# jmscraig/deequ

Measured on AMD Instinct MI355X. Metric: rows/sec + achieved HBM GB/s, fused 10-analyzer suite on 1B rows, 1/2/4/8 GPUs, higher is better.
Workload: dtype int64; 1 GPU; S10 fused suite (Size, Completeness(id), Completeness(name), Compliance(numViews >= 0), Compliance(priority IS NULL OR priority IN ('high','low')), Sum/Mean/StandardDeviation/Minimum/Maximum(numViews)) over a synthetic Item table: int64 id/numViews, string name/priority, 5% nulls (BASELINE.json configs[1]); rows_per_gpu=1000000000, batch_rows=67108864, parallelism=dp1

## Files before the change

### deequ_amd/csrc/api.cpp

```cpp
#include <hip/hip_runtime.h>

#include <algorithm>
#include <cmath>
#include <cstdarg>
#include <cstdio>
#include <cstdlib>
#include <cstring>
#include <map>
#include <mutex>
#include <memory>
#include <string>
#include <tuple>
#include <vector>

#include "decimal.h"
#include "engine.h"
#include "kernels.h"
#include "jfmt.h"

using namespace dq;

#include <atomic>
static std::atomic<long long> g_host_waits{0};
static hipError_t host_wait(hipStream_t st) {
// ... 391 lines not shown
  int op = n.op;
  auto is_lit = [](const Node* x) { return x->op == DQ_X_I64 || x->op == DQ_X_F64; };
  auto colref = [&](const Node* x) -> int {
    if (x->op == DQ_X_COL && is_numeric(types[x->col])) return x->col;
    return -1;
  };
  if (colref(b) >= 0 && is_lit(a)) {
    std::swap(a, b);
    op = flip_cmp(op);
  }
  int c = colref(a);
  if (c < 0 || !is_lit(b)) return false;
  out.col = c;
  out.op = op;
  out.lit_f64 = b->op == DQ_X_F64;
  out.li = b->i;
  out.ld = b->op == DQ_X_F64 ? b->d : (double)b->i;
  return true;
}

static bool fuse_numeric(const Node& n, const std::vector<int32_t>& types, int& col, NumPred& p) {
  p = NumPred{};
  if (interpreter_only(n)) return false;
  const Node* body = &n;
  int null_col = -1;
  if (n.op == DQ_X_OR && n.kids[0]->op == DQ_X_IS_NULL && n.kids[0]->kids[0]->op == DQ_X_COL) {
    null_col = n.kids[0]->kids[0]->col;
    body = n.kids[1].get();
  }
  CmpLeaf a, b;
  bool two = false;
  if (body->op == DQ_X_AND) {
    if (!leaf_cmp(*body->kids[0], types, a) || !leaf_cmp(*body->kids[1], types, b)) return false;
    if (a.col != b.col) return false;
    two = true;
  } else if (!leaf_cmp(*body, types, a)) {
    return false;
  }
  if (null_col >= 0 && null_col != a.col) return false;
  const bool fcol = is_floating(types[a.col]);
  const bool as_double = fcol || a.lit_f64 || (two && b.lit_f64);
  if (two && !fcol && (a.lit_f64 != b.lit_f64)) return false;
  if (as_double && !fcol && types[a.col] == DQ_INT64) {
  }
  col = a.col;
  p.op1 = a.op;
  p.op2 = two ? b.op : 0;
  p.as_double = as_double ? 1 : 0;
  p.null_is_true = null_col >= 0 ? 1 : 0;
  p.lo_i = a.li;
  p.lo_d = a.ld;
  p.hi_i = two ? b.li : 0;
  p.hi_d = two ? b.ld : 0.0;
  return true;
}

struct StrIn {
  int col = -1;
  bool negate = false;
  bool null_is_true = false;
  std::vector<std::string> list;
};

static bool fuse_str_in_body(const Node& n, const std::vector<int32_t>& types, StrIn& s) {
  if (n.op == DQ_X_NOT) {
    if (!fuse_str_in_body(*n.kids[0], types, s)) return false;
    s.negate = !s.negate;
    return true;
  }
  if (n.op == DQ_X_IN) {
    const Node& x = *n.kids[0];
    if (x.op != DQ_X_COL || types[x.col] != DQ_UTF8) return false;
    for (size_t k = 1; k < n.kids.size(); ++k) {
      if (n.kids[k]->op != DQ_X_STR) return false;
      s.list.push_back(n.kids[k]->s);
    }
    s.col = x.col;
    return true;
  }
  if (n.op == DQ_X_EQ || n.op == DQ_X_NE) {
    const Node* a = n.kids[0].get();
    const Node* b = n.kids[1].get();
    if (a->op == DQ_X_STR) std::swap(a, b);
    if (a->op != DQ_X_COL || types[a->col] != DQ_UTF8 || b->op != DQ_X_STR) return false;
    s.col = a->col;
    s.list.push_back(b->s);
    s.negate = n.op == DQ_X_NE;
    return true;
  }
  return false;
}

static bool fuse_str_in(const Node& n, const std::vector<int32_t>& types, StrIn& s) {
  s = StrIn{};
  if (interpreter_only(n)) return false;
  if (n.op == DQ_X_OR && n.kids[0]->op == DQ_X_IS_NULL && n.kids[0]->kids[0]->op == DQ_X_COL) {
    int nc = n.kids[0]->kids[0]->col;
    if (!fuse_str_in_body(*n.kids[1], types, s)) return false;
    if (s.col != nc) return false;
    s.null_is_true = true;
    return true;
  }
  return fuse_str_in_body(n, types, s);
}

enum SlotSrc { SRC_ROWS = 1, SRC_TASK = 2 };
// ... 338 lines not shown
  s += line;
  size_t n = std::min(buf_len - 1, s.size());
  memcpy(buf, s.data(), n);
  buf[n] = '\0';
  return DQ_OK;
}

extern "C" int dq_plan_launches_per_batch(const dq_plan* plan) {
  if (!plan) return 0;
  int classes = 0, hll = 0;
  for (int c = 0; c < kBodyClasses; ++c) {
    bool used = false;
    for (const TaskPlan& t : plan->tasks) used = used || (body_class(plan, t) == c && !t.carried);
    if (c == BC_HLL || c == BC_CORR_HLL || c == BC_DECIMAL) hll += used ? 1 : 0;
    else classes += used ? 1 : 0;
  }
  bool hll_alone = false;
  for (const TaskPlan& t : plan->tasks) hll_alone = hll_alone || (t.kind == TK_HLL && !t.carried);
  if (hll_alone && plan->n_hll <= kMixedHllMax && classes >= 1) {
    classes += 1;
    hll -= 1;
  }
  if (classes >= 2 && !getenv("DQ_NO_MIXED")) classes = 1;
  return (int)plan->mat.size() + classes + hll + (plan->tasks.empty() ? 0 : 1);
}

struct dq_state {
  const dq_plan* plan = nullptr;
  int device = 0;
  int grid[kQueues] = {};
  int mix_hll = 0;
  hipStream_t stream = nullptr;
  bool stream_set = false;
  std::vector<Acc> acc;
  std::vector<uint8_t> hll;
  int64_t rows = 0;
  bool host_dirty = false;
  bool reset_pending = false;
  bool synced = true;
  void* h_pin = nullptr;
  size_t h_pin_cap = 0;
  bool pin_pending = false;
  DevBuf<Acc> d_acc, d_partial, d_partial2;
  DevBuf<uint8_t> d_hll;
  DevBuf<uint32_t> d_hll_stage;
  DevBuf<uint32_t> d_fin_arrivals;
  DevBuf<int64_t> d_rows;
  DevBuf<int32_t> d_kinds;
  std::vector<int32_t> h_kinds;
  bool kinds_ready = false;
  hipEvent_t ev_xchg = nullptr;
  bool rows_on_device = false;
  DevBuf<uint32_t> d_queue;
  DevBuf<uint32_t> d_order[2];
  std::vector<uint32_t> order_sig[2];
  std::vector<size_t> order_off[2], order_len[2];
  uint32_t* h_order[2] = {nullptr, nullptr};
  size_t h_order_cap[2] = {0, 0};
  DevBuf<TaskDesc> d_tasks[2];
  TaskDesc* h_tasks[2] = {nullptr, nullptr};
  size_t h_tasks_cap[2] = {0, 0};
  hipEvent_t ev[2] = {nullptr, nullptr};
  bool ev_used[2] = {false, false};
  int flip = 0;
  DevBuf<uint64_t> d_bitmaps;
  size_t bitmap_words = 0;
  DevBuf<XInstr> d_prog;
  std::vector<int> prog_off;
  DevBuf<uint8_t> d_pool;
  std::vector<int64_t> pool_off;
  struct RegexRun {
    int col = -1, null_mode = 0, ns = 0, start = 0;
    int64_t table_off = 0;
  };
  std::vector<RegexRun> rx;
  DevBuf<DevCol> d_cols[2];
  DevCol* h_cols[2] = {nullptr, nullptr};
  size_t h_cols_cap[2] = {0, 0};
  DevBuf<int32_t> d_list_i32;
  DevBuf<uint64_t> d_list_pre;
  DevBuf<uint8_t> d_list_bytes;
  std::vector<int64_t> list_i32_base, list_pre_base, list_byte_base;
  ~dq_state() {
    for (int k = 0; k < 2; ++k) {
      if (h_tasks[k]) (void)hipHostFree(h_tasks[k]);
      if (h_cols[k]) (void)hipHostFree(h_cols[k]);
      if (h_order[k]) (void)hipHostFree(h_order[k]);
      if (ev[k]) (void)hipEventDestroy(ev[k]);
    }
    if (ev_xchg) (void)hipEventDestroy(ev_xchg);
  }
};

static void host_reset(dq_state* s) {
  const dq_plan* p = s->plan;
  s->acc.assign(p->tasks.size(), Acc{});
  for (size_t k = 0; k < p->tasks.size(); ++k) acc_init(p->tasks[k].kind, s->acc[k]);
  s->hll.assign((size_t)p->n_hll * kHllM, 0);
  s->rows = 0;
  s->host_dirty = true;
  s->synced = true;
}

static dq_status pin_ensure(dq_state* s, size_t bytes) {
  if (s->h_pin_cap >= bytes) return DQ_OK;
  if (s->pin_pending) {
    HIP_TRY(host_wait(s->stream));
    s->pin_pending = false;
  }
  if (s->h_pin) (void)hipHostFree(s->h_pin);
// ... 243 lines not shown
    }
    if (!ref[c]) continue;
    if (cols[c].length < 0) {
      st = fail(DQ_ERR_INVALID_ARGUMENT, "negative column length");
      return -1;
    }
    if (rows < 0) rows = cols[c].length;
    else if (rows != cols[c].length) {
      st = fail(DQ_ERR_INVALID_ARGUMENT, "columns of one batch differ in length");
      return -1;
    }
    if (cols[c].length > 0 && !cols[c].values) {
      st = fail(DQ_ERR_INVALID_ARGUMENT, "column %zu has no values buffer", c);
      return -1;
    }
    if (cols[c].type == DQ_UTF8 && cols[c].length > 0 && !cols[c].data) {
      st = fail(DQ_ERR_INVALID_ARGUMENT, "utf8 column %zu has no data buffer", c);
      return -1;
    }
  }
  if (rows < 0) rows = plan->types.empty() ? 0 : cols[0].length;
  if (rows > ((int64_t)1 << 40)) {
    st = fail(DQ_ERR_UNSUPPORTED, "batch too large");
    return -1;
  }
  return rows;
}

extern "C" dq_status dq_scan_device(const dq_plan* plan, const dq_column* cols, int n_cols,
                                    dq_state* s, void* hip_stream) {
  return dq_scan_device_batches(plan, cols, n_cols, 1, s, hip_stream);
}

constexpr int64_t kTailDiv = 32;
constexpr int64_t kTailCut = 8;
constexpr int64_t kTailMinItems = 16;
static bool tail_split() {
  static const bool on = [] {
    const char* e = getenv("DQ_TAIL_SPLIT");
    return !e || atoi(e) != 0;
  }();
  return on;
}

static bool scan_has_tail(const TaskDesc* td, size_t n_desc, const ScanLaunch& L) {
  for (size_t q = 0; q < n_desc; ++q)
    if (td[q].n_items > td[q].n_big && (uint32_t)td[q].item_begin >= L.item_lo &&
        (uint32_t)td[q].item_begin < L.item_hi)
      return true;
  return false;
}

static void scan_order(const TaskDesc* td, size_t n_desc, const std::vector<ScanLaunch>& G,
                       std::vector<uint32_t>& out) {
  std::vector<std::vector<uint32_t>> big(G.size()), small(G.size());
  for (size_t c = 0; c < G.size(); ++c)
    for (size_t q = 0; q < n_desc; ++q) {
      const TaskDesc& t = td[q];
      if (t.n_items == 0 || (uint32_t)t.item_begin < G[c].item_lo || (uint32_t)t.item_begin >= G[c].item_hi)
        continue;
      for (int64_t i = 0; i < t.n_items; ++i)
        (i < t.n_big ? big[c] : small[c]).push_back((uint32_t)(t.item_begin + i));
    }
  auto interleave = [](std::vector<std::vector<uint32_t>>& lists) {
    std::vector<uint32_t> r;
    std::vector<size_t> next(lists.size(), 0);
    size_t total = 0;
    for (auto& l : lists) total += l.size();
    r.reserve(total);
    for (size_t k = 0; k < total; ++k) {
      int best = -1;
      double best_key = 0.0;
      for (size_t c = 0; c < lists.size(); ++c) {
        if (next[c] >= lists[c].size()) continue;
        const double key = (next[c] + 0.5) / (double)lists[c].size();
        if (best < 0 || key < best_key) {
          best = (int)c;
          best_key = key;
        }
      }
      r.push_back(lists[best][next[best]++]);
    }
    return r;
  };
  const std::vector<uint32_t> B = interleave(big), S = interleave(small);
  const uint64_t n = B.size() + S.size();
  size_t bi = 0, si = 0;
  for (int x = 0; x < kQueueHeads; ++x) {
    const uint64_t len = n * (x + 1) / kQueueHeads - n * x / kQueueHeads;
    const uint64_t want_s = (uint64_t)S.size() * (x + 1) / kQueueHeads - (uint64_t)si;
    uint64_t ns = std::min<uint64_t>(want_s, len), nb = len - ns;
    if (nb > B.size() - bi) {
      nb = B.size() - bi;
      ns = len - nb;
    }
    for (uint64_t k = 0; k < nb; ++k) out.push_back(B[bi++]);
    for (uint64_t k = 0; k < ns; ++k) out.push_back(S[si++]);
  }
}

extern "C" dq_status dq_scan_device_batches(const dq_plan* plan, const dq_column* cols, int n_cols,
                                            int n_batches, dq_state* s, void* hip_stream) {
  if (!plan || !s || (n_cols > 0 && n_batches > 0 && !cols))
    return fail(DQ_ERR_INVALID_ARGUMENT, "null argument");
  if (n_batches < 0) return fail(DQ_ERR_INVALID_ARGUMENT, "negative batch count");
  if (s->plan != plan) return fail(DQ_ERR_STATE, "state was created for another plan");
  if (n_cols < (int)plan->types.size())
    return fail(DQ_ERR_NO_SUCH_COLUMN, "plan needs %zu columns, got %d", plan->types.size(), n_cols);
  if (n_batches == 0) return DQ_OK;
  if (s->device < 0) return fail(DQ_ERR_STATE, "host-only state (device -1) cannot scan");
  hipStream_t stream = reinterpret_cast<hipStream_t>(hip_stream);
  HIP_TRY(hipSetDevice(s->device));
  if (s->rows_on_device) {
    const dq_status rs = dq_state_sync(s);
    if (rs != DQ_OK) return rs;
  }
  if (s->stream_set && s->stream != stream) HIP_TRY(host_wait(s->stream));
  s->stream = stream;
  s->stream_set = true;
  dq_status st = upload_host(s);
  if (st != DQ_OK) return st;

  std::vector<int> ref(plan->types.size(), 0);
  for (const TaskPlan& t : plan->tasks) {
    if (t.col >= 0) ref[t.col] = 1;
    if (t.col2 >= 0) ref[t.col2] = 1;
  }
  for (const MatExpr& m : plan->mat)
    for (const XInstr& ins : m.prog)
      if (ins.op == XI_COL) ref[ins.a] = 1;
  std::vector<int64_t> rows(n_batches);
  int64_t total_rows = 0;
  for (int b = 0; b < n_batches; ++b) {
    rows[b] = batch_rows(plan, cols + (size_t)b * n_cols, ref, st);
    if (rows[b] < 0) return st;
    total_rows += rows[b];
  }

// ... 157 lines not shown
      item_rows = std::max<int64_t>(kItemAlign, std::min<int64_t>(item_rows, (int64_t)1 << 22));
      t.item_rows = item_rows;
      t.n_items = rows[b] > 0 && !tp.carried ? (rows[b] + item_rows - 1) / item_rows : 0;
      t.n_big = t.n_items;
      t.small_rows = item_rows;
      if (tail_split() && t.n_items >= kTailMinItems && item_rows >= kTailCut * kItemAlign) {
        const int64_t k = (t.n_items + kTailDiv - 1) / kTailDiv;
        t.n_big = t.n_items - k;
        t.small_rows = item_rows / kTailCut;
        t.n_items = t.n_big + (rows[b] - t.n_big * item_rows + t.small_rows - 1) / t.small_rows;
      }
      t.item_begin = total_items;
      total_items += t.n_items;
      td[d] = t;
    }
    const int c = body_class(plan, tp);
    if (launches.empty() || launches.back().body != c)
      launches.push_back(ScanLaunch{c, s->grid[c], (uint32_t)td[d - n_batches].item_begin, 0, nullptr});
    launches.back().item_hi = (uint32_t)total_items;
  }
  if (total_items >= ((int64_t)1 << 31))
    return fail(DQ_ERR_UNSUPPORTED, "scan of %lld work items exceeds one launch",
                (long long)total_items);
  {
    std::vector<ScanLaunch> plain, hll;
    for (const ScanLaunch& L : launches)
      ((L.body == BC_HLL && !s->mix_hll) || L.body == BC_CORR_HLL || L.body == BC_DECIMAL ? hll : plain)
          .push_back(L);
    const bool mixed = plain.size() >= 2 && !getenv("DQ_NO_MIXED");
    if (mixed && plain.front().item_lo != 0) return fail(DQ_ERR_STATE, "unexpected item layout");
    std::vector<std::vector<ScanLaunch>> groups;
    if (mixed) groups.push_back(plain);
    else
      for (const ScanLaunch& L : plain) groups.push_back({L});
    for (const ScanLaunch& L : hll) groups.push_back({L});
    std::vector<uint32_t> sig;
    for (size_t q = 0; q < n_desc; ++q) {
      sig.push_back((uint32_t)td[q].item_begin);
      sig.push_back((uint32_t)td[q].n_big);
      sig.push_back((uint32_t)td[q].n_items);
    }
    for (const auto& G : groups) {
      sig.push_back(0xffffffffu);
      for (const ScanLaunch& L : G) {
        sig.push_back(L.item_lo);
        sig.push_back(L.item_hi);
      }
    }
    std::vector<size_t>& off = s->order_off[slot];
    std::vector<size_t>& len = s->order_len[slot];
    if (s->order_sig[slot] != sig) {
      off.assign(groups.size(), 0);
      len.assign(groups.size(), 0);
      std::vector<uint32_t> all;
      for (size_t g = 0; g < groups.size(); ++g) {
        off[g] = all.size();
        if (groups[g].size() >= 2 || scan_has_tail(td, n_desc, groups[g][0])) {
          scan_order(td, n_desc, groups[g], all);
          len[g] = all.size() - off[g];
        }
      }
      HIP_TRY(s->d_order[slot].ensure(std::max<size_t>(1, all.size())));
      if (!all.empty()) {
        if (s->h_order_cap[slot] < all.size()) {
          if (s->h_order[slot]) HIP_TRY(hipHostFree(s->h_order[slot]));
          s->h_order[slot] = nullptr;
          s->h_order_cap[slot] = 0;
          HIP_TRY(hipHostMalloc((void**)&s->h_order[slot], all.size() * sizeof(uint32_t),
                                hipHostMallocDefault));
          s->h_order_cap[slot] = all.size();
        }
        memcpy(s->h_order[slot], all.data(), all.size() * sizeof(uint32_t));
        HIP_TRY(hipMemcpyAsync(s->d_order[slot].p, s->h_order[slot], all.size() * sizeof(uint32_t),
                               hipMemcpyHostToDevice, stream));
      }
      s->order_sig[slot] = sig;
    }
    launches.clear();
    for (size_t g = 0; g < groups.size(); ++g) {
      const uint32_t* ord = len[g] ? s->d_order[slot].p + off[g] : nullptr;
      if (groups[g].size() >= 2) {
        bool has_hll = false;
        uint32_t classes = 0;
        for (const ScanLaunch& L : groups[g]) {
          has_hll = has_hll || L.body == BC_HLL;
          classes |= 1u << L.body;
        }
        launches.push_back(ScanLaunch{kBodyMixed, s->grid[kBodyMixed], 0, (uint32_t)len[g], ord,
                                      has_hll ? s->mix_hll : 0, classes});
      } else {
        ScanLaunch L = groups[g][0];
        if (ord) {
          L.item_lo = 0;
          L.item_hi = (uint32_t)len[g];
          L.order = ord;
        }
        launches.push_back(L);
      }
    }
  }
  if (getenv("DQ_DEBUG")) {
    for (const ScanLaunch& L : launches)
      fprintf(stderr, "[dq] launch body=%d grid=%d items=[%u,%u)\n", L.body, L.grid, L.item_lo,
              L.item_hi);
    for (size_t q = 0; q < n_desc; ++q)
      fprintf(stderr, "[dq] desc %zu kind=%d out=%d rows=%lld item_rows=%lld items=[%lld,+%lld) vec=%d\n",
              q, td[q].kind, td[q].out, (long long)td[q].rows, (long long)td[q].item_rows,
              (long long)td[q].item_begin, (long long)td[q].n_items, td[q].vec_ok);
  }
  if (n_desc > 0 && total_items > 0) {
    HIP_TRY(s->d_partial.ensure((size_t)total_items));
    HIP_TRY(hipMemcpyAsync(s->d_tasks[slot].p, td, n_desc * sizeof(TaskDesc), hipMemcpyHostToDevice,
                           stream));
    HIP_TRY(launch_scan(s->d_tasks[slot].p, (int)n_desc, (int)plan->tasks.size(), launches.data(),
                        (int)launches.size(), plan->n_hll, s->d_queue.p, s->d_partial.p,
                        s->d_partial2.p, s->d_hll_stage.p, s->d_acc.p, s->d_hll.p,
                        s->d_fin_arrivals.p, stream, s->reset_pending ? 1 : 0));
    s->reset_pending = false;
    s->synced = false;
  }
  HIP_TRY(hipEventRecord(s->ev[slot], stream));
  s->ev_used[slot] = true;
  s->rows += total_rows;
  return DQ_OK;
}

extern "C" dq_status dq_state_sync(dq_state* s) {
  if (!s) return fail(DQ_ERR_INVALID_ARGUMENT, "null state");
  if (s->synced || s->device < 0) return DQ_OK;
  HIP_TRY(hipSetDevice(s->device));
  const size_t ab = s->acc.size() * sizeof(Acc), hb = s->hll.size();
  const size_t rb = s->rows_on_device ? 8 : 0;
  {
// ... 817 lines not shown
```

### deequ_amd/csrc/engine.h

```cpp
#pragma once

#include <hip/hip_runtime.h>
#include <stdint.h>

#include "../../include/deequ_amd.h"

#define DQ_HD __host__ __device__ __forceinline__

namespace dq {

enum TaskKind : int32_t {
  TK_NUMERIC = 1,
  TK_VALIDITY = 2,
  TK_STR_IN = 3,
  TK_BOOLMAP = 4,
  TK_COMOMENTS = 5,
  TK_HLL = 6,
  TK_DTYPE = 7,
  TK_DECIMAL = 8
};

constexpr int kMaxPreds = 3;
constexpr int kHllP = 9;
constexpr int kHllM = 1 << kHllP;
constexpr int kHllWords = 52;
constexpr int kHllRegsPerWord = 10;
constexpr int kHllRegBits = 6;
constexpr int kBlock = 256;
constexpr int kWaveRows = 1024;
#ifndef DQ_ITEM_BYTES
#define DQ_ITEM_BYTES 262144
#endif
constexpr double kItemBytes = DQ_ITEM_BYTES;
constexpr int kItemAlign = 1024;
constexpr int kFinParts = 32;
constexpr int kListLenSlots = 65;

struct NumPred {
  int32_t op1, op2;
  int32_t as_double;
  int32_t null_is_true;
  int64_t lo_i, hi_i;
  double lo_d, hi_d;
};

struct TaskDesc {
  int32_t kind, type, type2, n_preds;
  int32_t out;
  int32_t hll_out;
  int32_t batch;
  int32_t negate;
  int32_t null_is_true;
  int32_t n_list;
  int32_t vec_ok;
  int32_t list_small;
  int32_t body;
  int32_t hll_side;
  uint64_t list_lenmask;
  uint64_t list_key[8];
  int64_t rows;
  int64_t item_rows;
  int64_t item_begin;
  int64_t n_items;
  int64_t n_big;
  int64_t small_rows;
  const uint8_t* valid;
  const void* values;
  const uint8_t* data;
  const uint8_t* valid2;
  const void* values2;
  const uint8_t* w_val;
  const uint8_t* w_vld;
  const uint8_t* b_val;
  const uint8_t* b_vld;
  const int32_t* list_start;
  const int32_t* list_len;
  const int32_t* list_boff;
  const uint64_t* list_pre;
  const uint8_t* list_bytes;
  NumPred preds[kMaxPreds];
};

struct alignas(16) Acc {
  int64_t i[10];
  double d[6];
};

DQ_HD void acc_init(int kind, Acc& a) {
  for (int k = 0; k < 10; ++k) a.i[k] = 0;
  for (int k = 0; k < 6; ++k) a.d[k] = 0.0;
  if (kind == TK_NUMERIC) {
    a.i[2] = INT64_MAX;
    a.i[3] = INT64_MIN;
  }
  if (kind == TK_DECIMAL) {
    a.i[4] = -1;
    a.i[5] = INT64_MAX;
// ... 288 lines not shown
```

### deequ_amd/csrc/kernels.h

```cpp
#pragma once

#include <hip/hip_runtime.h>
#include <stdint.h>

#include <string>
#include <utility>
#include <vector>

#include "engine.h"

namespace dq {

dq_status fail(dq_status code, const char* fmt, ...);

#define HIP_TRY(expr)                                                                        \
  do {                                                                                       \
    hipError_t _e = (expr);                                                                  \
    if (_e != hipSuccess) {                                                                  \
      return ::dq::fail(_e == hipErrorOutOfMemory ? DQ_ERR_OUT_OF_MEMORY : DQ_ERR_DEVICE,    \
                        "HIP error %s (%d) at %s:%d", hipGetErrorString(_e), (int)_e,        \
                        __FILE__, __LINE__);                                                 \
    }                                                                                        \
  } while (0)

// ... 86 lines not shown
  LK_ENDS,
  LK_ALL
};

struct XInstr {
  int32_t op;
  int32_t a;
  int64_t imm;
};

constexpr int kMaxStack = 16;

hipError_t launch_bitmap_rebase(const uint8_t* src, int64_t bit, int64_t rows, uint8_t* dst,
                                hipStream_t stream);
hipError_t launch_tile_scan(uint32_t* tiles, int64_t n, hipStream_t stream);
bool dict_index_type_ok(int index_type);
hipError_t launch_dict_count(const void* indices, int index_type, const uint8_t* valid, int64_t rows,
                             int64_t entries, unsigned long long* counts, unsigned long long* words,
                             hipStream_t stream);
hipError_t launch_expr(const XInstr* prog, int n_instr, const DevCol* cols, const uint8_t* pool,
                       int64_t rows, uint64_t* out_val, uint64_t* out_vld, hipStream_t stream);
constexpr int kRegexMaxStates = 255;
hipError_t launch_regex(const uint8_t* valid, const int32_t* offsets, const uint8_t* data,
                        int64_t rows, const uint8_t* table, int ns, int start, int null_mode,
                        uint64_t* out_val, uint64_t* out_vld, hipStream_t stream);
bool build_regex_table(const std::string& pool, int64_t at, std::vector<uint8_t>& tab, int* ns_out,
                       int* start_out);
enum BodyClass : int32_t {
  BC_NUM_I8 = 0,
  BC_NUM_I16,
  BC_NUM_I32,
  BC_NUM_I64,
  BC_NUM_F32,
  BC_NUM_F64,
  BC_BITS,
  BC_STR_IN,
  BC_DTYPE,
  BC_CORR,
  BC_HLL,
  BC_CORR_HLL,
  BC_DECIMAL,
  kBodyClasses
};
constexpr int kBodyMixed = kBodyClasses;
constexpr int kQueues = kBodyClasses + 1;
constexpr int kQueueHeads = 8;
constexpr int kQueueStride = 32;
constexpr int kQueueWords = kQueues * kQueueHeads * kQueueStride;

struct ScanLaunch {
  int32_t body;
  int32_t grid;
  uint32_t item_lo, item_hi;
  const uint32_t* order;
  int32_t lds_hll = 0;
  uint32_t classes = 0;
};
constexpr uint32_t kMixedAll = ((1u << kBodyClasses) - 1u) & ~(1u << BC_DECIMAL);
constexpr uint32_t kMixedS10 = (1u << BC_BITS) | (1u << BC_NUM_I64) | (1u << BC_STR_IN);

constexpr int kMixedHllMax = 0;

hipError_t launch_scan(const TaskDesc* tasks, int n_desc, int n_tasks, const ScanLaunch* launches,
                       int n_launches, int n_hll, uint32_t* queues, Acc* partial, Acc* partial2,
                       uint32_t* hll_stage, Acc* acc, uint8_t* hll_acc, uint32_t* arrivals,
                       hipStream_t stream, int reset = 0);
size_t scan_lds_bytes(int body, int n_hll);
int scan_max_blocks_per_cu(int body, int n_hll);
void plan_column_needs(const dq_plan* plan, std::vector<int>& need);

}
```

### deequ_amd/csrc/scan.hip

```cpp
#include <hip/hip_runtime.h>

#include <cstdlib>

#include "device_util.h"
#include "kernels.h"
#include "stream_load.h"

namespace dq {

DQ_DEV void wave_reduce(int kind, Acc& a) {
#pragma unroll
  for (int off = 32; off > 0; off >>= 1) {
    Acc o;
#pragma unroll
    for (int f = 0; f < 10; ++f) o.i[f] = __shfl_xor(a.i[f], off);
#pragma unroll
    for (int f = 0; f < 6; ++f) o.d[f] = __shfl_xor(a.d[f], off);
    acc_merge(kind, a, o);
  }
}

DQ_DEV uint32_t ld32_slow(const uint8_t* bm, int64_t word, int64_t rows) {
  if (!bm) return 0xffffffffu;
  uint32_t v = 0;
  for (int b = 0; b < 4; ++b) {
    int64_t byte = word * 4 + b;
    if (byte * 8 < rows) v |= (uint32_t)bm[byte] << (8 * b);
  }
  return v;
}

DQ_DEV bool near_constant(double m2b, int nb, double mb) {
  return m2b <= (double)nb * (mb * mb) * 0x1p-88;
}

template <int N, typename T>
DQ_DEV bool clamp_block_mean(const T* x, uint32_t sel, double& mb) {
  double lo = INFINITY, hi = -INFINITY;
#pragma unroll
  for (int i = 0; i < N; ++i) {
    const bool on = (sel >> i) & 1u;
    const double xd = (double)x[i];
    lo = (on && xd < lo) ? xd : lo;
    hi = (on && xd > hi) ? xd : hi;
  }
  const double c = mb < lo ? lo : (mb > hi ? hi : mb);
  const bool moved = c != mb;
  mb = c;
  return moved;
}

struct NumLane {
  int64_t n = 0, si = 0, kmin = INT64_MAX, kmax = INT64_MIN;
  double sd = 0.0, mean = 0.0, m2 = 0.0;
  uint32_t pt[kMaxPreds] = {0, 0, 0}, pn[kMaxPreds] = {0, 0, 0};
};

template <typename T>
DQ_DEV int64_t num_key(T v) {
  if constexpr (std::is_floating_point<T>::value) {
    return f64_key((double)v);
  } else {
    return (int64_t)v;
  }
}

template <typename T, int NV>
DQ_DEV uint32_t pred_bits(const NumPred& P, const T* x) {
  const uint32_t m1 = op_mask(P.op1), m2 = op_mask(P.op2);
  uint32_t r = 0;
  if (P.as_double) {
    const double lo = P.lo_d, hi = P.hi_d;
#pragma unroll
    for (int i = 0; i < NV; ++i) {
      const double xd = (double)x[i];
      uint32_t ok = (m1 >> (cmp3_f64(xd, lo) + 1)) & 1u;
      if (P.op2) ok &= (m2 >> (cmp3_f64(xd, hi) + 1)) & 1u;
      r |= ok << i;
    }
  } else {
    const int64_t lo = P.lo_i, hi = P.hi_i;
#pragma unroll
    for (int i = 0; i < NV; ++i) {
      const int64_t xi = (int64_t)x[i];
      uint32_t ok = (m1 >> (cmp3_i64(xi, lo) + 1)) & 1u;
      if (P.op2) ok &= (m2 >> (cmp3_i64(xi, hi) + 1)) & 1u;
      r |= ok << i;
    }
  }
  return r;
}

template <typename T, int NV>
DQ_DEV void num_vals(NumLane& L, const T* x, uint32_t vb, uint32_t wt, const TaskDesc& t) {
  const uint32_t sel = vb & wt;
  const int nb = __popc(sel);
  if (nb) {
    double s = 0.0;
#pragma unroll
    for (int i = 0; i < NV; ++i) {
      const bool on = (sel >> i) & 1u;
      if constexpr (!std::is_floating_point<T>::value) L.si = wrap_add(L.si, on ? (int64_t)x[i] : 0);
      s += on ? (double)x[i] : 0.0;
      const int64_t k = num_key(x[i]);
      L.kmin = (on && k < L.kmin) ? k : L.kmin;
      L.kmax = (on && k > L.kmax) ? k : L.kmax;
    }
    if constexpr (std::is_floating_point<T>::value) L.sd += s;
    double mb = s / (double)nb;
    double m2b = 0.0;
#pragma unroll
    for (int i = 0; i < NV; ++i) {
      const double d = (double)x[i] - mb;
      m2b += ((sel >> i) & 1u) ? d * d : 0.0;
    }
    if (near_constant(m2b, nb, mb) && clamp_block_mean<NV>(x, sel, mb)) {
      m2b = 0.0;
#pragma unroll
      for (int i = 0; i < NV; ++i) {
        const double d = (double)x[i] - mb;
        m2b += ((sel >> i) & 1u) ? d * d : 0.0;
      }
    }
    if (L.n == 0) {
      L.mean = mb;
      L.m2 = m2b;
    } else {
      moments_merge((double)L.n, L.mean, L.m2, (double)nb, mb, m2b);
    }
    L.n += nb;
  }
  if (t.n_preds == 0) return;
  const uint32_t nulls_all = wt & ~vb & ((1u << NV) - 1u);
#pragma unroll
  for (int p = 0; p < kMaxPreds; ++p) {
    if (p >= t.n_preds) break;
    const NumPred& P = t.preds[p];
    const uint32_t r = pred_bits<T, NV>(P, x);
    const uint32_t nulls = P.null_is_true ? nulls_all : 0u;
    L.pt[p] += __popc(r & sel) + __popc(nulls);
    L.pn[p] += __popc(sel) + __popc(nulls);
  }
}

template <typename T>
DQ_DEV void num_rows(NumLane& L, const T (&x)[16], uint32_t vb, uint32_t wt, const TaskDesc& t) {
  num_vals<T, 8>(L, x, vb & 0xffu, wt & 0xffu, t);
  num_vals<T, 8>(L, x + 8, vb >> 8, wt >> 8, t);
}

template <typename T>
DQ_DEV void num_chunk_fast(NumLane& L, const TaskDesc& t, int64_t r0) {
  constexpr int VPL = 16 / (int)sizeof(T);
  constexpr int U = 16 / VPL;
  const int l = lane_id();
  const T* v = reinterpret_cast<const T*>(t.values) + r0;
  uint4 raw[U];
#pragma unroll
  for (int k = 0; k < U; ++k) raw[k] = ld16(v + (k * 64 + l) * VPL);
  uint32_t vb = 0xffffu, wt = 0xffffu;
  if (t.valid) {
    ChunkBits c;
    c.load(t.valid, r0);
    vb = 0;
#pragma unroll
    for (int k = 0; k < U; ++k) vb |= c.get((k * 64 + l) * VPL, VPL) << (k * VPL);
  }
  if (t.w_val) {
    ChunkBits a, b;
    a.load(t.w_val, r0);
    b.load(t.w_vld, r0);
    wt = 0;
#pragma unroll
    for (int k = 0; k < U; ++k) {
      const int o = (k * 64 + l) * VPL;
      wt |= (a.get(o, VPL) & b.get(o, VPL)) << (k * VPL);
    }
  }
  T x[16];
  __builtin_memcpy(x, raw, sizeof(x));
  num_rows<T>(L, x, vb, wt, t);
}

template <typename T>
DQ_DEV void num_chunk_slow(NumLane& L, const TaskDesc& t, int64_t r0, int64_t r_end) {
  constexpr int VPL = 16 / (int)sizeof(T);
  constexpr int U = 16 / VPL;
  const int l = lane_id();
  const T* v = reinterpret_cast<const T*>(t.values);
#pragma unroll 1
  for (int k = 0; k < U; ++k) {
    T x[VPL];
    uint32_t vb = 0, wt = 0;
#pragma unroll
    for (int j = 0; j < VPL; ++j) {
      const int64_t r = r0 + (int64_t)(k * 64 + l) * VPL + j;
      x[j] = T(0);
      if (r < r_end) {
        x[j] = v[r];
        vb |= bit1(t.valid, r) << j;
        const uint32_t w = t.w_val ? (bit1(t.w_val, r) & bit1(t.w_vld, r)) : 1u;
        wt |= w << j;
      }
    }
    num_vals<T, VPL>(L, x, vb, wt, t);
  }
}

template <typename T>
DQ_DEV void num_item(const TaskDesc& t, int64_t r_begin, int64_t r_end, Acc& a) {
  NumLane L;
  int64_t r0 = r_begin;
  if (t.vec_ok)
    for (; r0 + kWaveRows <= r_end; r0 += kWaveRows) num_chunk_fast<T>(L, t, r0);
  for (; r0 < r_end; r0 += kWaveRows) num_chunk_slow<T>(L, t, r0, r_end);
  a.i[0] = L.n;
  a.i[1] = L.si;
  a.i[2] = L.kmin;
  a.i[3] = L.kmax;
#pragma unroll
  for (int p = 0; p < kMaxPreds; ++p) {
    a.i[4 + p] = L.pt[p];
    a.i[7 + p] = L.pn[p];
  }
  a.d[0] = L.sd;
  a.d[1] = L.mean;
  a.d[2] = L.m2;
}

DQ_DEV void bits_item(const TaskDesc& t, int64_t r_begin, int64_t r_end, Acc& acc) {
  const uint8_t* A = t.kind == TK_VALIDITY ? t.valid : t.b_val;
  const uint8_t* B = t.kind == TK_VALIDITY ? nullptr : t.b_vld;
  const uint8_t* WV = t.w_val;
  const uint8_t* WD = t.w_val ? t.w_vld : nullptr;
  const int l = lane_id();
  int64_t c0 = 0, c1 = 0;
  int64_t r0 = r_begin;
  if (t.vec_ok) {
    const uint4 ones = make_uint4(~0u, ~0u, ~0u, ~0u);
    for (; r0 + 32768 <= r_end; r0 += 32768) {
      uint4 a[4], b[4], x[4], y[4];
#pragma unroll
      for (int k = 0; k < 4; ++k) {
        const int64_t byte = (r0 >> 3) + 1024 * k + 16 * l;
        a[k] = A ? ld16(A + byte) : ones;
        b[k] = B ? ld16(B + byte) : ones;
        x[k] = WV ? ld16(WV + byte) : ones;
        y[k] = WD ? ld16(WD + byte) : ones;
      }
#pragma unroll
      for (int k = 0; k < 4; ++k) {
        const uint32_t m0 = b[k].x & x[k].x & y[k].x, m1 = b[k].y & x[k].y & y[k].y,
                       m2 = b[k].z & x[k].z & y[k].z, m3 = b[k].w & x[k].w & y[k].w;
        c0 += __popc(a[k].x & m0) + __popc(a[k].y & m1) + __popc(a[k].z & m2) +
              __popc(a[k].w & m3);
        c1 += __popc(m0) + __popc(m1) + __popc(m2) + __popc(m3);
      }
    }
    for (; r0 + 8192 <= r_end; r0 += 8192) {
      const int64_t byte = (r0 >> 3) + 16 * l;
      const uint4 a = A ? ld16(A + byte) : ones;
      const uint4 b = B ? ld16(B + byte) : ones;
      const uint4 x = WV ? ld16(WV + byte) : ones;
      const uint4 y = WD ? ld16(WD + byte) : ones;
      const uint32_t m0 = b.x & x.x & y.x, m1 = b.y & x.y & y.y, m2 = b.z & x.z & y.z,
                     m3 = b.w & x.w & y.w;
      c0 += __popc(a.x & m0) + __popc(a.y & m1) + __popc(a.z & m2) + __popc(a.w & m3);
// ... 646 lines not shown
    const uint32_t vx = bits32(t.valid, w), vy = bits32(t.valid2, w);
    const uint32_t wm = t.w_val ? bits32(t.w_val, w) & bits32(t.w_vld, w) : ~0u;
    sel |= (((vx & vy & wm) >> sh) & 3u) << (2 * k);
    hsel |= ((((hy ? vy : vx) & wm) >> sh) & 3u) << (2 * k);
  }
#pragma unroll
  for (int k = 0; k < K; ++k) {
    const uint4 q = hy ? qy[k] : qx[k];
    uint64_t x0 = (uint64_t)q.x | ((uint64_t)q.y << 32);
    uint64_t x1 = (uint64_t)q.z | ((uint64_t)q.w << 32);
    if (hdbl) {
      if (__builtin_bit_cast(double, x0) != __builtin_bit_cast(double, x0)) x0 = 0x7ff8000000000000ULL;
      if (__builtin_bit_cast(double, x1) != __builtin_bit_cast(double, x1)) x1 = 0x7ff8000000000000ULL;
    }
    const uint64_t h0 = xxh_long(x0, 42), h1 = xxh_long(x1, 42);
    if ((hsel >> (2 * k)) & 1u) hll_update(regs, h0);
    if ((hsel >> (2 * k + 1)) & 1u) hll_update(regs, h1);
  }
  corr_fold16<K>(qx, qy, sel, xl, yl, n, c);
}

DQ_DEV void item_range(const TaskDesc& t, uint32_t item, int64_t& r_begin, int64_t& r_end) {
  const int64_t li = (int64_t)item - t.item_begin;
  if (li < t.n_big) {
    r_begin = li * t.item_rows;
    r_end = min(r_begin + t.item_rows, t.rows);
  } else {
    r_begin = t.n_big * t.item_rows + (li - t.n_big) * t.small_rows;
    r_end = min(r_begin + t.small_rows, t.rows);
  }
}

DQ_DEV bool queue_next(uint32_t* heads, uint32_t lo, uint32_t hi, int home, int& step,
                       uint32_t& item) {
  const uint32_t n = hi - lo;
  while (step < kQueueHeads) {
    const int x = (home + step) % kQueueHeads;
    const uint32_t b = lo + (uint32_t)((uint64_t)n * x / kQueueHeads);
    const uint32_t e = lo + (uint32_t)((uint64_t)n * (x + 1) / kQueueHeads);
    uint32_t v = 0;
    if (b < e) {
      if (lane_id() == 0) v = atomicAdd(&heads[x * kQueueStride], 1u);
      v = __builtin_amdgcn_readfirstlane(v);
      if (v < e - b) {
        item = b + v;
        return true;
      }
    }
    ++step;
  }
  return false;
}

template <int BC, int K = 8>
__global__ void __launch_bounds__(kBlock, (BC == BC_CORR_HLL ? (K == 8 ? 4 : 5) : 1)) scan_kernel(const TaskDesc* __restrict__ tasks, int n_desc,
                                                      uint32_t item_lo, uint32_t item_hi,
                                                      const uint32_t* __restrict__ order,
                                                      uint32_t* __restrict__ queue,
                                                      Acc* __restrict__ partial,
                                                      uint32_t* __restrict__ hll_stage, int n_hll) {
  extern __shared__ uint32_t hll_lds[];
  constexpr bool kRegs = BC == BC_HLL || BC == BC_CORR_HLL;
  if constexpr (kRegs) {
    for (int i = threadIdx.x; i < n_hll * kHllM; i += kBlock) hll_lds[i] = 0;
    __syncthreads();
  }
  const int l = lane_id();
  int step = 0;
  uint32_t item = 0;
  while (queue_next(queue, item_lo, item_hi, (int)(blockIdx.x % kQueueHeads), step, item)) {
    if (order) item = order[item];
    int lo = 0, hi = n_desc - 1;
    while (lo < hi) {
      const int mid = (lo + hi + 1) >> 1;
      if ((uint64_t)tasks[mid].item_begin <= item) lo = mid;
      else hi = mid - 1;
    }
    const TaskDesc& t = tasks[lo];
    int64_t r_begin, r_end;
    item_range(t, item, r_begin, r_end);
    Acc a;
    acc_init(t.kind, a);
    if constexpr (BC == BC_NUM_I8) num_item<int8_t>(t, r_begin, r_end, a);
    if constexpr (BC == BC_NUM_I16) num_item<int16_t>(t, r_begin, r_end, a);
    if constexpr (BC == BC_NUM_I32) num_item<int32_t>(t, r_begin, r_end, a);
    if constexpr (BC == BC_NUM_I64) num_item<int64_t>(t, r_begin, r_end, a);
    if constexpr (BC == BC_NUM_F32) num_item<float>(t, r_begin, r_end, a);
    if constexpr (BC == BC_NUM_F64) num_item<double>(t, r_begin, r_end, a);
    if constexpr (BC == BC_BITS) bits_item(t, r_begin, r_end, a);
    if constexpr (BC == BC_STR_IN) str_in_item(t, r_begin, r_end, a);
    if constexpr (BC == BC_DTYPE) dtype_item(t, r_begin, r_end, a);
    if constexpr (BC == BC_CORR) corr_item(t, r_begin, r_end, a);
    if constexpr (BC == BC_DECIMAL) dec_item(t, r_begin, r_end, a);
    if constexpr (BC == BC_CORR_HLL) corr_rows<true, K>(t, r_begin, r_end, a, hll_lds + t.hll_out * kHllM);
    if constexpr (BC == BC_HLL) {
      hll_item(t, r_begin, r_end, hll_lds + t.hll_out * kHllM);
    } else {
      constexpr int kind = BC <= BC_NUM_F64 ? TK_NUMERIC
                           : BC == BC_BITS  ? TK_VALIDITY
                           : BC == BC_DTYPE ? TK_DTYPE
                           : BC == BC_CORR || BC == BC_CORR_HLL ? TK_COMOMENTS
                           : BC == BC_DECIMAL ? TK_DECIMAL
                                            : TK_STR_IN;
      wave_reduce(kind, a);
      if (l == 0) partial[item] = a;
    }
  }
  if constexpr (kRegs) {
    __syncthreads();
    for (int i = threadIdx.x; i < n_hll * kHllM; i += kBlock) {
      const uint32_t v = hll_lds[i];
      if (v) atomicMax(&hll_stage[i], v);
    }
  }
}

static_assert(kMixedHllMax == 0, "scan_mixed_kernel has no HLL body");

template <uint32_t MASK>
__global__ void __launch_bounds__(kBlock) __attribute__((amdgpu_waves_per_eu(3, 3)))
scan_mixed_kernel(const TaskDesc* __restrict__ tasks, int n_desc, uint32_t n_order,
                  const uint32_t* __restrict__ order, uint32_t* __restrict__ queue,
                  Acc* __restrict__ partial, uint32_t* __restrict__ hll_stage, int n_hll) {
  extern __shared__ uint32_t mix_lds[];
  if (n_hll) {
    for (int i = threadIdx.x; i < n_hll * kHllM; i += kBlock) mix_lds[i] = 0;
    __syncthreads();
  }
  const int l = lane_id();
  int step = 0;
  uint32_t q = 0;
  while (queue_next(queue, 0, n_order, (int)(blockIdx.x % kQueueHeads), step, q)) {
    const uint32_t item = order[q];
    int lo = 0, hi = n_desc - 1;
    while (lo < hi) {
      const int mid = (lo + hi + 1) >> 1;
      if ((uint64_t)tasks[mid].item_begin <= item) lo = mid;
      else hi = mid - 1;
    }
    const TaskDesc& t = tasks[lo];
    int64_t r_begin, r_end;
    item_range(t, item, r_begin, r_end);
    Acc a;
    acc_init(t.kind, a);
#define DQ_BODY(BCV, CALL) \
  case BCV:                \
    if constexpr ((MASK >> BCV) & 1u) CALL; \
    break;
    switch (t.body) {
      DQ_BODY(BC_NUM_I8, (num_item<int8_t>(t, r_begin, r_end, a)))
      DQ_BODY(BC_NUM_I16, (num_item<int16_t>(t, r_begin, r_end, a)))
      DQ_BODY(BC_NUM_I32, (num_item<int32_t>(t, r_begin, r_end, a)))
      DQ_BODY(BC_NUM_I64, (num_item<int64_t>(t, r_begin, r_end, a)))
      DQ_BODY(BC_NUM_F32, (num_item<float>(t, r_begin, r_end, a)))
      DQ_BODY(BC_NUM_F64, (num_item<double>(t, r_begin, r_end, a)))
      DQ_BODY(BC_BITS, (bits_item(t, r_begin, r_end, a)))
      DQ_BODY(BC_STR_IN, (str_in_item(t, r_begin, r_end, a)))
      DQ_BODY(BC_DTYPE, (dtype_item(t, r_begin, r_end, a)))
      DQ_BODY(BC_CORR, (corr_item(t, r_begin, r_end, a)))
      default: break;
    }
#undef DQ_BODY
    wave_reduce(t.kind, a);
    if (l == 0) partial[item] = a;
  }
  if (n_hll) {
    __syncthreads();
    for (int i = threadIdx.x; i < n_hll * kHllM; i += kBlock) {
      const uint32_t v = mix_lds[i];
      if (v) atomicMax(&hll_stage[i], v);
    }
  }
}

DQ_DEV void task_range_block(const TaskDesc* tasks, int n_desc, int task, int64_t& lo, int64_t& hi,
                             int& kind, int& hll_out) {
  __shared__ unsigned long long s_lo, s_hi;
  __shared__ int s_kind, s_hll;
  if (threadIdx.x == 0) {
    s_lo = ~0ULL;
    s_hi = 0;
    s_kind = 0;
    s_hll = -1;
  }
  __syncthreads();
  for (int d = threadIdx.x; d < n_desc; d += blockDim.x) {
    const TaskDesc& t = tasks[d];
    if (t.out != task) continue;
    atomicMin(&s_lo, (unsigned long long)t.item_begin);
    atomicMax(&s_hi, (unsigned long long)(t.item_begin + t.n_items));
    s_kind = t.kind;
    s_hll = t.hll_out;
  }
  __syncthreads();
  lo = s_lo == ~0ULL ? 0 : (int64_t)s_lo;
  hi = s_lo == ~0ULL ? 0 : (int64_t)s_hi;
  kind = s_kind;
  hll_out = s_hll;
  __syncthreads();
}

DQ_DEV void wave_merge_tree(int kind, Acc& a) {
#pragma unroll
  for (int s = 32; s > 0; s >>= 1) {
    Acc b;
#pragma unroll
    for (int k = 0; k < 10; ++k) b.i[k] = __shfl_down(a.i[k], s);
#pragma unroll
    for (int k = 0; k < 6; ++k) b.d[k] = __shfl_down(a.d[k], s);
    if (lane_id() < s) acc_merge(kind, a, b);
  }
}

__global__ void __launch_bounds__(kBlock) finalize_kernel(const TaskDesc* __restrict__ tasks,
                                                          int n_desc,
                                                          const Acc* __restrict__ partial,
// ... 181 lines not shown
```

Before: 347.1 billion rows/s.

## Specialize predicate forms, pack descriptor index into order, trim wave reductions

Integer predicates of a simple form are classified on the host and evaluated with compile-time-specialized comparison code, and single-predicate numeric loops are templated on that form. Scan order entries grow to 64 bits and carry the task descriptor index, so kernels no longer binary-search the descriptor table per item. Wave reductions are templated on the accumulator kind and shuffle only the fields that kind uses. The costs are doubled order-buffer traffic, more kernel instantiations and code size, and reliance on per-kind field counts being correct.

```diff
diff --git a/deequ_amd/csrc/api.cpp b/deequ_amd/csrc/api.cpp
--- a/deequ_amd/csrc/api.cpp
+++ b/deequ_amd/csrc/api.cpp
@@ -467,6 +467,7 @@
   p.lo_d = a.ld;
   p.hi_i = two ? b.li : 0;
   p.hi_d = two ? b.ld : 0.0;
+  p.form = pred_form(p);
   return true;
 }
 
@@ -911,10 +912,10 @@
   hipEvent_t ev_xchg = nullptr;
   bool rows_on_device = false;
   DevBuf<uint32_t> d_queue;
-  DevBuf<uint32_t> d_order[2];
+  DevBuf<uint64_t> d_order[2];
   std::vector<uint32_t> order_sig[2];
   std::vector<size_t> order_off[2], order_len[2];
-  uint32_t* h_order[2] = {nullptr, nullptr};
+  uint64_t* h_order[2] = {nullptr, nullptr};
   size_t h_order_cap[2] = {0, 0};
   DevBuf<TaskDesc> d_tasks[2];
   TaskDesc* h_tasks[2] = {nullptr, nullptr};
@@ -1264,18 +1265,19 @@
 }
 
 static void scan_order(const TaskDesc* td, size_t n_desc, const std::vector<ScanLaunch>& G,
-                       std::vector<uint32_t>& out) {
-  std::vector<std::vector<uint32_t>> big(G.size()), small(G.size());
+                       std::vector<uint64_t>& out) {
+  std::vector<std::vector<uint64_t>> big(G.size()), small(G.size());
   for (size_t c = 0; c < G.size(); ++c)
     for (size_t q = 0; q < n_desc; ++q) {
       const TaskDesc& t = td[q];
       if (t.n_items == 0 || (uint32_t)t.item_begin < G[c].item_lo || (uint32_t)t.item_begin >= G[c].item_hi)
         continue;
       for (int64_t i = 0; i < t.n_items; ++i)
-        (i < t.n_big ? big[c] : small[c]).push_back((uint32_t)(t.item_begin + i));
-    }
-  auto interleave = [](std::vector<std::vector<uint32_t>>& lists) {
-    std::vector<uint32_t> r;
+        (i < t.n_big ? big[c] : small[c])
+            .push_back((uint64_t)(uint32_t)(t.item_begin + i) | ((uint64_t)q << 32));
+    }
+  auto interleave = [](std::vector<std::vector<uint64_t>>& lists) {
+    std::vector<uint64_t> r;
     std::vector<size_t> next(lists.size(), 0);
     size_t total = 0;
     for (auto& l : lists) total += l.size();
@@ -1295,7 +1297,7 @@
     }
     return r;
   };
-  const std::vector<uint32_t> B = interleave(big), S = interleave(small);
+  const std::vector<uint64_t> B = interleave(big), S = interleave(small);
   const uint64_t n = B.size() + S.size();
   size_t bi = 0, si = 0;
   for (int x = 0; x < kQueueHeads; ++x) {
@@ -1559,7 +1561,7 @@
     if (s->order_sig[slot] != sig) {
       off.assign(groups.size(), 0);
       len.assign(groups.size(), 0);
-      std::vector<uint32_t> all;
+      std::vector<uint64_t> all;
       for (size_t g = 0; g < groups.size(); ++g) {
         off[g] = all.size();
         if (groups[g].size() >= 2 || scan_has_tail(td, n_desc, groups[g][0])) {
@@ -1573,19 +1575,19 @@
           if (s->h_order[slot]) HIP_TRY(hipHostFree(s->h_order[slot]));
           s->h_order[slot] = nullptr;
           s->h_order_cap[slot] = 0;
-          HIP_TRY(hipHostMalloc((void**)&s->h_order[slot], all.size() * sizeof(uint32_t),
+          HIP_TRY(hipHostMalloc((void**)&s->h_order[slot], all.size() * sizeof(uint64_t),
                                 hipHostMallocDefault));
           s->h_order_cap[slot] = all.size();
         }
-        memcpy(s->h_order[slot], all.data(), all.size() * sizeof(uint32_t));
-        HIP_TRY(hipMemcpyAsync(s->d_order[slot].p, s->h_order[slot], all.size() * sizeof(uint32_t),
+        memcpy(s->h_order[slot], all.data(), all.size() * sizeof(uint64_t));
+        HIP_TRY(hipMemcpyAsync(s->d_order[slot].p, s->h_order[slot], all.size() * sizeof(uint64_t),
                                hipMemcpyHostToDevice, stream));
       }
       s->order_sig[slot] = sig;
     }
     launches.clear();
     for (size_t g = 0; g < groups.size(); ++g) {
-      const uint32_t* ord = len[g] ? s->d_order[slot].p + off[g] : nullptr;
+      const uint64_t* ord = len[g] ? s->d_order[slot].p + off[g] : nullptr;
       if (groups[g].size() >= 2) {
         bool has_hll = false;
         uint32_t classes = 0;
diff --git a/deequ_amd/csrc/engine.h b/deequ_amd/csrc/engine.h
--- a/deequ_amd/csrc/engine.h
+++ b/deequ_amd/csrc/engine.h
@@ -36,13 +36,42 @@
 constexpr int kFinParts = 32;
 constexpr int kListLenSlots = 65;
 
+enum PredForm : int32_t {
+  PF_GENERIC = 0,
+  PF_I_EQ,
+  PF_I_NE,
+  PF_I_LT,
+  PF_I_LE,
+  PF_I_GT,
+  PF_I_GE,
+  PF_I_BETWEEN
+};
+
 struct NumPred {
   int32_t op1, op2;
   int32_t as_double;
   int32_t null_is_true;
   int64_t lo_i, hi_i;
   double lo_d, hi_d;
-};
+  int32_t form;
+  int32_t pad;
+};
+
+inline int32_t pred_form(const NumPred& p) {
+  if (p.as_double) return PF_GENERIC;
+  if (p.op2 == 0) {
+    switch (p.op1) {
+      case DQ_X_EQ: return PF_I_EQ;
+      case DQ_X_NE: return PF_I_NE;
+      case DQ_X_LT: return PF_I_LT;
+      case DQ_X_LE: return PF_I_LE;
+      case DQ_X_GT: return PF_I_GT;
+      case DQ_X_GE: return PF_I_GE;
+      default: return PF_GENERIC;
+    }
+  }
+  return p.op1 == DQ_X_GE && p.op2 == DQ_X_LE ? PF_I_BETWEEN : PF_GENERIC;
+}
 
 struct TaskDesc {
   int32_t kind, type, type2, n_preds;
diff --git a/deequ_amd/csrc/kernels.h b/deequ_amd/csrc/kernels.h
--- a/deequ_amd/csrc/kernels.h
+++ b/deequ_amd/csrc/kernels.h
@@ -162,7 +162,7 @@
   int32_t body;
   int32_t grid;
   uint32_t item_lo, item_hi;
-  const uint32_t* order;
+  const uint64_t* order;
   int32_t lds_hll = 0;
   uint32_t classes = 0;
 };
diff --git a/deequ_amd/csrc/scan.hip b/deequ_amd/csrc/scan.hip
--- a/deequ_amd/csrc/scan.hip
+++ b/deequ_amd/csrc/scan.hip
@@ -8,15 +8,19 @@
 
 namespace dq {
 
-DQ_DEV void wave_reduce(int kind, Acc& a) {
+template <int KIND>
+DQ_DEV void wave_reduce(Acc& a) {
+  constexpr int NI = KIND == TK_NUMERIC ? 10 : KIND == TK_DECIMAL ? 8 : KIND == TK_DTYPE ? 5
+                     : KIND == TK_COMOMENTS ? 1 : 2;
+  constexpr int ND = KIND == TK_NUMERIC || KIND == TK_DECIMAL ? 3 : KIND == TK_COMOMENTS ? 5 : 0;
 #pragma unroll
   for (int off = 32; off > 0; off >>= 1) {
-    Acc o;
-#pragma unroll
-    for (int f = 0; f < 10; ++f) o.i[f] = __shfl_xor(a.i[f], off);
-#pragma unroll
-    for (int f = 0; f < 6; ++f) o.d[f] = __shfl_xor(a.d[f], off);
-    acc_merge(kind, a, o);
+    Acc o = a;
+#pragma unroll
+    for (int f = 0; f < NI; ++f) o.i[f] = __shfl_xor(a.i[f], off);
+#pragma unroll
+    for (int f = 0; f < ND; ++f) o.d[f] = __shfl_xor(a.d[f], off);
+    acc_merge(KIND, a, o);
   }
 }
 
@@ -66,7 +70,7 @@
 }
 
 template <typename T, int NV>
-DQ_DEV uint32_t pred_bits(const NumPred& P, const T* x) {
+DQ_DEV uint32_t pred_bits_generic(const NumPred& P, const T* x) {
   const uint32_t m1 = op_mask(P.op1), m2 = op_mask(P.op2);
   uint32_t r = 0;
   if (P.as_double) {
@@ -91,7 +95,49 @@
   return r;
 }
 
+template <int FORM, typename T, int NV>
+DQ_DEV uint32_t pred_bits_form(const NumPred& P, const T* x) {
+  if constexpr (FORM == PF_GENERIC || std::is_floating_point<T>::value) {
+    return pred_bits_generic<T, NV>(P, x);
+  } else {
+    const int64_t lo = P.lo_i, hi = P.hi_i;
+    uint32_t r = 0;
+#pragma unroll
+    for (int i = 0; i < NV; ++i) {
+      const int64_t xi = (int64_t)x[i];
+      bool ok;
+      if constexpr (FORM == PF_I_EQ) ok = xi == lo;
+      if constexpr (FORM == PF_I_NE) ok = xi != lo;
+      if constexpr (FORM == PF_I_LT) ok = xi < lo;
+      if constexpr (FORM == PF_I_LE) ok = xi <= lo;
+      if constexpr (FORM == PF_I_GT) ok = xi > lo;
+      if constexpr (FORM == PF_I_GE) ok = xi >= lo;
+      if constexpr (FORM == PF_I_BETWEEN) ok = xi >= lo && xi <= hi;
+      r |= (ok ? 1u : 0u) << i;
+    }
+    return r;
+  }
+}
+
 template <typename T, int NV>
+DQ_DEV uint32_t pred_bits(const NumPred& P, const T* x) {
+  switch (P.form) {
+    case PF_I_EQ: return pred_bits_form<PF_I_EQ, T, NV>(P, x);
+    case PF_I_NE: return pred_bits_form<PF_I_NE, T, NV>(P, x);
+    case PF_I_LT: return pred_bits_form<PF_I_LT, T, NV>(P, x);
+    case PF_I_LE: return pred_bits_form<PF_I_LE, T, NV>(P, x);
+    case PF_I_GT: return pred_bits_form<PF_I_GT, T, NV>(P, x);
+    case PF_I_GE: return pred_bits_form<PF_I_GE, T, NV>(P, x);
+    case PF_I_BETWEEN: return pred_bits_form<PF_I_BETWEEN, T, NV>(P, x);
+    default: return pred_bits_generic<T, NV>(P, x);
+  }
+}
+
+constexpr int kPredsNone = -1;
+constexpr int kPredsAny = -2;
+constexpr int kPredsGeneric = -3;
+
+template <typename T, int NV, int PM = kPredsAny>
 DQ_DEV void num_vals(NumLane& L, const T* x, uint32_t vb, uint32_t wt, const TaskDesc& t) {
   const uint32_t sel = vb & wt;
   const int nb = __popc(sel);
@@ -130,26 +176,34 @@
     }
     L.n += nb;
   }
-  if (t.n_preds == 0) return;
+  if constexpr (PM == kPredsNone) return;
   const uint32_t nulls_all = wt & ~vb & ((1u << NV) - 1u);
-#pragma unroll
-  for (int p = 0; p < kMaxPreds; ++p) {
-    if (p >= t.n_preds) break;
-    const NumPred& P = t.preds[p];
-    const uint32_t r = pred_bits<T, NV>(P, x);
+  if constexpr (PM >= 0) {
+    const NumPred& P = t.preds[0];
+    const uint32_t r = pred_bits_form<PM, T, NV>(P, x);
     const uint32_t nulls = P.null_is_true ? nulls_all : 0u;
-    L.pt[p] += __popc(r & sel) + __popc(nulls);
-    L.pn[p] += __popc(sel) + __popc(nulls);
-  }
-}
-
-template <typename T>
+    L.pt[0] += __popc(r & sel) + __popc(nulls);
+    L.pn[0] += __popc(sel) + __popc(nulls);
+  } else {
+#pragma unroll
+    for (int p = 0; p < kMaxPreds; ++p) {
+      if (p >= t.n_preds) break;
+      const NumPred& P = t.preds[p];
+      const uint32_t r = PM == kPredsGeneric ? pred_bits_generic<T, NV>(P, x) : pred_bits<T, NV>(P, x);
+      const uint32_t nulls = P.null_is_true ? nulls_all : 0u;
+      L.pt[p] += __popc(r & sel) + __popc(nulls);
+      L.pn[p] += __popc(sel) + __popc(nulls);
+    }
+  }
+}
+
+template <typename T, int PM>
 DQ_DEV void num_rows(NumLane& L, const T (&x)[16], uint32_t vb, uint32_t wt, const TaskDesc& t) {
-  num_vals<T, 8>(L, x, vb & 0xffu, wt & 0xffu, t);
-  num_vals<T, 8>(L, x + 8, vb >> 8, wt >> 8, t);
-}
-
-template <typename T>
+  num_vals<T, 8, PM>(L, x, vb & 0xffu, wt & 0xffu, t);
+  num_vals<T, 8, PM>(L, x + 8, vb >> 8, wt >> 8, t);
+}
+
+template <typename T, int PM>
 DQ_DEV void num_chunk_fast(NumLane& L, const TaskDesc& t, int64_t r0) {
   constexpr int VPL = 16 / (int)sizeof(T);
   constexpr int U = 16 / VPL;
@@ -179,7 +233,7 @@
   }
   T x[16];
   __builtin_memcpy(x, raw, sizeof(x));
-  num_rows<T>(L, x, vb, wt, t);
+  num_rows<T, PM>(L, x, vb, wt, t);
 }
 
 template <typename T>
@@ -203,16 +257,39 @@
         wt |= w << j;
       }
     }
-    num_vals<T, VPL>(L, x, vb, wt, t);
-  }
-}
-
-template <typename T>
+    num_vals<T, VPL, kPredsGeneric>(L, x, vb, wt, t);
+  }
+}
+
+template <typename T, bool FORMS = true>
 DQ_DEV void num_item(const TaskDesc& t, int64_t r_begin, int64_t r_end, Acc& a) {
   NumLane L;
   int64_t r0 = r_begin;
-  if (t.vec_ok)
-    for (; r0 + kWaveRows <= r_end; r0 += kWaveRows) num_chunk_fast<T>(L, t, r0);
+  if (t.vec_ok) {
+    const int pm = t.n_preds == 0 ? kPredsNone
+                   : !FORMS          ? kPredsGeneric
+                   : t.n_preds == 1  ? t.preds[0].form
+                                     : kPredsAny;
+#define DQ_NUM_LOOP(PMV) \
+  case PMV:              \
+    for (; r0 + kWaveRows <= r_end; r0 += kWaveRows) num_chunk_fast<T, PMV>(L, t, r0); \
+    break;
+    switch (pm) {
+      DQ_NUM_LOOP(kPredsNone)
+      DQ_NUM_LOOP(PF_I_EQ)
+      DQ_NUM_LOOP(PF_I_NE)
+      DQ_NUM_LOOP(PF_I_LT)
+      DQ_NUM_LOOP(PF_I_LE)
+      DQ_NUM_LOOP(PF_I_GT)
+      DQ_NUM_LOOP(PF_I_GE)
+      DQ_NUM_LOOP(PF_I_BETWEEN)
+      default:
+        for (; r0 + kWaveRows <= r_end; r0 += kWaveRows)
+          num_chunk_fast<T, FORMS ? kPredsAny : kPredsGeneric>(L, t, r0);
+        break;
+    }
+#undef DQ_NUM_LOOP
+  }
   for (; r0 < r_end; r0 += kWaveRows) num_chunk_slow<T>(L, t, r0, r_end);
   a.i[0] = L.n;
   a.i[1] = L.si;
@@ -965,10 +1042,13 @@
   return false;
 }
 
+DQ_DEV uint32_t entry_item(uint64_t e) { return (uint32_t)e; }
+DQ_DEV int entry_desc(uint64_t e) { return (int)(e >> 32); }
+
 template <int BC, int K = 8>
 __global__ void __launch_bounds__(kBlock, (BC == BC_CORR_HLL ? (K == 8 ? 4 : 5) : 1)) scan_kernel(const TaskDesc* __restrict__ tasks, int n_desc,
                                                       uint32_t item_lo, uint32_t item_hi,
-                                                      const uint32_t* __restrict__ order,
+                                                      const uint64_t* __restrict__ order,
                                                       uint32_t* __restrict__ queue,
                                                       Acc* __restrict__ partial,
                                                       uint32_t* __restrict__ hll_stage, int n_hll) {
@@ -982,12 +1062,18 @@
   int step = 0;
   uint32_t item = 0;
   while (queue_next(queue, item_lo, item_hi, (int)(blockIdx.x % kQueueHeads), step, item)) {
-    if (order) item = order[item];
-    int lo = 0, hi = n_desc - 1;
-    while (lo < hi) {
-      const int mid = (lo + hi + 1) >> 1;
-      if ((uint64_t)tasks[mid].item_begin <= item) lo = mid;
-      else hi = mid - 1;
+    int lo = 0;
+    if (order) {
+      const uint64_t e = order[item];
+      item = entry_item(e);
+      lo = entry_desc(e);
+    } else {
+      int hi = n_desc - 1;
+      while (lo < hi) {
+        const int mid = (lo + hi + 1) >> 1;
+        if ((uint64_t)tasks[mid].item_begin <= item) lo = mid;
+        else hi = mid - 1;
+      }
     }
     const TaskDesc& t = tasks[lo];
     int64_t r_begin, r_end;
@@ -1015,7 +1101,7 @@
                            : BC == BC_CORR || BC == BC_CORR_HLL ? TK_COMOMENTS
                            : BC == BC_DECIMAL ? TK_DECIMAL
                                             : TK_STR_IN;
-      wave_reduce(kind, a);
+      wave_reduce<kind>(a);
       if (l == 0) partial[item] = a;
     }
   }
@@ -1033,7 +1119,7 @@
 template <uint32_t MASK>
 __global__ void __launch_bounds__(kBlock) __attribute__((amdgpu_waves_per_eu(3, 3)))
 scan_mixed_kernel(const TaskDesc* __restrict__ tasks, int n_desc, uint32_t n_order,
-                  const uint32_t* __restrict__ order, uint32_t* __restrict__ queue,
+                  const uint64_t* __restrict__ order, uint32_t* __restrict__ queue,
                   Acc* __restrict__ partial, uint32_t* __restrict__ hll_stage, int n_hll) {
   extern __shared__ uint32_t mix_lds[];
   if (n_hll) {
@@ -1044,14 +1130,9 @@
   int step = 0;
   uint32_t q = 0;
   while (queue_next(queue, 0, n_order, (int)(blockIdx.x % kQueueHeads), step, q)) {
-    const uint32_t item = order[q];
-    int lo = 0, hi = n_desc - 1;
-    while (lo < hi) {
-      const int mid = (lo + hi + 1) >> 1;
-      if ((uint64_t)tasks[mid].item_begin <= item) lo = mid;
-      else hi = mid - 1;
-    }
-    const TaskDesc& t = tasks[lo];
+    const uint64_t entry = order[q];
+    const uint32_t item = entry_item(entry);
+    const TaskDesc& t = tasks[entry_desc(entry)];
     int64_t r_begin, r_end;
     item_range(t, item, r_begin, r_end);
     Acc a;
@@ -1060,13 +1141,14 @@
   case BCV:                \
     if constexpr ((MASK >> BCV) & 1u) CALL; \
     break;
+    constexpr bool kForms = MASK == kMixedS10;
     switch (t.body) {
-      DQ_BODY(BC_NUM_I8, (num_item<int8_t>(t, r_begin, r_end, a)))
-      DQ_BODY(BC_NUM_I16, (num_item<int16_t>(t, r_begin, r_end, a)))
-      DQ_BODY(BC_NUM_I32, (num_item<int32_t>(t, r_begin, r_end, a)))
-      DQ_BODY(BC_NUM_I64, (num_item<int64_t>(t, r_begin, r_end, a)))
-      DQ_BODY(BC_NUM_F32, (num_item<float>(t, r_begin, r_end, a)))
-      DQ_BODY(BC_NUM_F64, (num_item<double>(t, r_begin, r_end, a)))
+      DQ_BODY(BC_NUM_I8, (num_item<int8_t, kForms>(t, r_begin, r_end, a)))
+      DQ_BODY(BC_NUM_I16, (num_item<int16_t, kForms>(t, r_begin, r_end, a)))
+      DQ_BODY(BC_NUM_I32, (num_item<int32_t, kForms>(t, r_begin, r_end, a)))
+      DQ_BODY(BC_NUM_I64, (num_item<int64_t, kForms>(t, r_begin, r_end, a)))
+      DQ_BODY(BC_NUM_F32, (num_item<float, kForms>(t, r_begin, r_end, a)))
+      DQ_BODY(BC_NUM_F64, (num_item<double, kForms>(t, r_begin, r_end, a)))
       DQ_BODY(BC_BITS, (bits_item(t, r_begin, r_end, a)))
       DQ_BODY(BC_STR_IN, (str_in_item(t, r_begin, r_end, a)))
       DQ_BODY(BC_DTYPE, (dtype_item(t, r_begin, r_end, a)))
@@ -1074,7 +1156,12 @@
       default: break;
     }
 #undef DQ_BODY
-    wave_reduce(t.kind, a);
+    switch (t.kind) {
+      case TK_NUMERIC: wave_reduce<TK_NUMERIC>(a); break;
+      case TK_DTYPE: wave_reduce<TK_DTYPE>(a); break;
+      case TK_COMOMENTS: wave_reduce<TK_COMOMENTS>(a); break;
+      default: wave_reduce<TK_VALIDITY>(a); break;
+    }
     if (l == 0) partial[item] = a;
   }
   if (n_hll) {
```

Measured after the change: 347.4 billion rows/s (median of 2 runs). No clear change (+0.1%).
